# mhamilton723/STEGO

Hardware: AMD Instinct MI355X
Metric: image-pairs/sec through correspondence loss, B=32 224^2, ViT-S/8 (higher is better)
Workload: dtype f16x3 (f32 inputs / outputs / accumulation; products of the feature and code correlations and of the backward's code GEMMs as fp16 hi+lo splits, 22-bit, on the matrix cores - error vs fp64 in the fp32 class, bounded by tests on adversarial inputs); 1 GPU; vits8_224: B=32/GPU, C=384, 28x28 map, K=70, S=11, 5 negatives, self+KNN+random correlation loss, forward+backward; global_batch=32, parallelism=dp1, launch=eager, input_sets_rotated=4, layout=channels-last strided views (as DinoFeaturizer)

## Files before the change

stego_amd/csrc/corr_bwd.hip:

```cpp
#include "corr_common.h"
#include "host_util.h"

namespace stego {

constexpr int LDG = 130;
constexpr int SMB_NRM = 0;
constexpr int SMB_AN = SMB_NRM + 2 * TP * 4;

template <int NT>
__device__ __forceinline__ void normalize_bwd_store(f32x4 (&d)[2][NT], const float* __restrict__ Cn, int ldk,
                                                    const float* __restrict__ nrm, float* __restrict__ dt_out,
                                                    int K, int KQ, int lane, int wave)
{
    const int cl = lane & 15, rg = lane >> 4;
#pragma unroll
    for (int mt = 0; mt < 2; ++mt) {
#pragma unroll
        for (int reg = 0; reg < 4; ++reg) {
            const int pt = 32 * wave + 16 * mt + 4 * rg + reg;
            float cn[NT];
            float dot = 0.f;
#pragma unroll
            for (int nt = 0; nt < NT; ++nt) {
                const int ch = 16 * nt + cl;
// ... 150 lines not shown
    if (!sameAB) normalize_bwd_store<NT>(dA, An, ldk, nrm, dtA, K, prm.KQ, lane, wave);
    for (int kk = 0; kk < kend; kk += 4) {
        const int k = kk + kq;
        float gt[2], an[NT];
        gt[0] = G[k * LDG + row0];
        gt[1] = G[k * LDG + row0 + 16];
#pragma unroll
        for (int nt = 0; nt < NT; ++nt) an[nt] = An[k * ldk + 16 * nt + cl];
#pragma unroll
        for (int nt = 0; nt < NT; ++nt) {
            dB[0][nt] = __builtin_amdgcn_mfma_f32_16x16x4f32(gt[0], an[nt], dB[0][nt], 0, 0, 0);
            dB[1][nt] = __builtin_amdgcn_mfma_f32_16x16x4f32(gt[1], an[nt], dB[1][nt], 0, 0, 0);
        }
    }
    if (stamp_on) ts[2] = __builtin_amdgcn_s_memrealtime();
    if (sameAB) {
#pragma unroll
        for (int mt = 0; mt < 2; ++mt)
#pragma unroll
            for (int nt = 0; nt < NT; ++nt) dA[mt][nt] += dB[mt][nt];
        normalize_bwd_store<NT>(dA, An, ldk, nrm, dtA, K, prm.KQ, lane, wave);
    } else {
        normalize_bwd_store<NT>(dB, Bn, ldk, nrm + TP, dtA + (size_t)TP * ldk, K, prm.KQ, lane, wave);
    }
    if (stamp_on) ts[3] = __builtin_amdgcn_s_memrealtime();
}

template <int NT>
__global__ void __launch_bounds__(NTHREADS) corr_bwd_tile_kernel(const BwdParams prm)
{
    extern __shared__ __attribute__((aligned(16))) unsigned char smem[];
    bwd_tile_body<NT>(prm, (int)blockIdx.x, smem);
}

constexpr int HB_LDR = 136;
constexpr int SMH_NRM = 0;
constexpr int SMH_CT = 1280;

typedef _Float16 f16x4 __attribute__((ext_vector_type(4)));

constexpr int HW_WAVES = 8;
constexpr int HW_THREADS = 64 * HW_WAVES;
constexpr int HW_NP = TP / (16 * HW_WAVES);
template <int NT>
__device__ __forceinline__ void normalize_bwd_store_t(f32x4 (&d)[NT][HW_NP], const float* __restrict__ Cn, int ldk,
                                                      const float* __restrict__ nrm, float* __restrict__ dt_out,
                                                      int K, int KQ, int lane, int wave, bool wt = false)
{
    const int cl = lane & 15, kq = lane >> 4;
#pragma unroll
    for (int np = 0; np < HW_NP; ++np) {
        const int pt = 16 * (HW_NP * wave + np) + cl;
        f32x4 cn[NT];
        float dot = 0.f;
#pragma unroll
        for (int mc = 0; mc < NT; ++mc) {
            const int ch0 = 16 * mc + 4 * kq;
            cn[mc] = *reinterpret_cast<const f32x4*>(Cn + (size_t)pt * ldk + ch0);
#pragma unroll
            for (int reg = 0; reg < 4; ++reg) {
                if (ch0 + reg >= K) cn[mc][reg] = 0.f;
                dot += cn[mc][reg] * (ch0 + reg < K ? d[mc][np][reg] : 0.f);
            }
        }
        dot += __shfl_xor(dot, 16, 64);
        dot += __shfl_xor(dot, 32, 64);
        const float nr = nrm[pt];
        const bool big = nr > 1e-10f;
        const float inv = 1.f / fmaxf(nr, 1e-10f);
#pragma unroll
        for (int mc = 0; mc < NT; ++mc) {
            const int ch0 = 16 * mc + 4 * kq;
            if (ch0 < KQ) {
                f32x4 v;
#pragma unroll
                for (int reg = 0; reg < 4; ++reg) {
                    const float dn = d[mc][np][reg];
                    v[reg] = big ? (dn - cn[mc][reg] * dot) * inv : dn * inv;
                    if (ch0 + reg >= K) v[reg] = 0.f;
                }
                float* dst = dt_out + (size_t)pt * ldk + ch0;
                if (wt) asm volatile("global_store_dwordx4 %0, %1, off sc1" :: "v"(dst), "v"(v) : "memory");
                else *reinterpret_cast<f32x4*>(dst) = v;
            }
        }
    }
}

template <int NT, bool DENSE>
__device__ __forceinline__ void bwd_tile_h_body(const BwdParams& prm, const int tile, unsigned char* smem)
{
    constexpr int NTG = NT <= 5 ? NT : (NT + 1) / 2;
    constexpr int NG = (NT + NTG - 1) / NTG;
    constexpr int CTR = 16 * NTG;
    float* nrm = reinterpret_cast<float*>(smem + SMH_NRM);
    float* red = nrm + 2 * TP;
    half_t* CT = reinterpret_cast<half_t*>(smem + SMH_CT);
    half_t* Gh = CT + 4 * CTR * HB_LDR;
    half_t* Gl = Gh + TP * HB_LDR;

    const int tid = threadIdx.x, lane = tid & 63;
    const int wave = __builtin_amdgcn_readfirstlane(tid >> 6);
    const int B = prm.B, P = prm.P, K = prm.K, ldk = prm.LDK;
    const int b = tile % B, p = tile / B;
    const bool sameAB = p == 0;
    const int sA = b;
    const int sB = p == 0 ? b : p * B + b;
    const float* csA = prm.cs + (size_t)sA * TP * ldk;
    const float* csB = prm.cs + (size_t)sB * TP * ldk;

    unsigned long long* ts = reinterpret_cast<unsigned long long*>(prm.dt + (size_t)prm.n_sets * B * 2 * TP * ldk) + 4096 + (size_t)tile * 4;
    const bool stamp_on = (prm.debug & 8) && tid == 0 && tile < 1024;
    if (stamp_on) ts[0] = __builtin_amdgcn_s_memrealtime();

    const int P2 = P * P;
    const size_t t0 = p < 2 ? (size_t)b * P2 : ((size_t)(p - 2) * B + b) * P2;
    const float* wp = prm.saved_w + ((size_t)p * B + b) * P2;
    const float* glp = wp;
    bool has_gl = false;
    float gl_b = 0.f;
    if (p >= 2) {
        if (prm.g_neg_loss) {
            if (DENSE && prm.g_neg_loss_stride > 0) { glp = prm.g_neg_loss + t0; has_gl = true; }
            else if (prm.g_neg_loss_stride < 0) gl_b = prm.g_neg_loss[0] * (1.f / ((float)B * (float)P2 * (float)prm.n_neg));
            else gl_b = prm.g_neg_loss[0];
        }
    } else {
        const float* gs = p == 0 ? prm.g_intra : prm.g_inter;
        if (gs) gl_b = gs[0] * (1.f / ((float)B * (float)P2));
    }
    const float* gcd = !DENSE ? nullptr : (p == 0 ? prm.g_intra_cd : (p == 1 ? prm.g_inter_cd : prm.g_neg_cd));
    const bool has_gc = gcd != nullptr;
    const float* gcp = has_gc ? gcd + t0 : wp;
    const float om = prm.saved_mean[p];

    constexpr int RB = TP / HW_WAVES;
    constexpr int c4n = CTR / 4;
    constexpr int NIT = ((TP / 2) * c4n + HW_THREADS - 1) / HW_THREADS;
    float wv[RB][2], glv[RB][2], gcv[RB][2];
    f32x4 r0[2][NIT], r1[2][NIT];
    auto load_codes = [&](int grp) {
#pragma unroll
        for (int side = 0; side < 2; ++side) {
            const float* src = ((side == 0 || sameAB) ? csA : csB) + grp * CTR;
#pragma unroll
            for (int it = 0; it < NIT; ++it) {
                const int i = (prm.debug & 16) ? 0 : min(tid + it * HW_THREADS, (TP / 2) * c4n - 1);
                const int pp = i / c4n, c4 = i - pp * c4n;
                r0[side][it] = *reinterpret_cast<const f32x4*>(src + (size_t)(2 * pp) * ldk + 4 * c4);
                r1[side][it] = *reinterpret_cast<const f32x4*>(src + (size_t)(2 * pp + 1) * ldk + 4 * c4);
            }
        }
    };
    auto convert_codes = [&](int grp) {
#pragma unroll
        for (int side = 0; side < 2; ++side) {
            if (side == 1 && sameAB) break;
            half_t* dh = CT + (size_t)(2 * side) * CTR * HB_LDR;
            half_t* dl = dh + CTR * HB_LDR;
#pragma unroll
            for (int it = 0; it < NIT; ++it) {
                const int i = tid + it * HW_THREADS;
                if (i < (TP / 2) * c4n) {
                    const int pp = i / c4n, c4 = i - pp * c4n;
#pragma unroll
                    for (int e = 0; e < 4; ++e) {
                        const int ch = 4 * c4 + e;
                        const bool in = grp * CTR + ch < K;
                        unsigned h, l;
                        split_f16_pair(in ? r0[side][it][e] : 0.f, in ? r1[side][it][e] : 0.f, h, l);
                        const int col = (((pp >> 1) ^ (ch >> 4)) << 2) + 2 * (pp & 1);
                        *reinterpret_cast<unsigned*>(dh + ch * HB_LDR + col) = h;
                        *reinterpret_cast<unsigned*>(dl + ch * HB_LDR + col) = l;
                    }
                }
            }
        }
    };
    {
        const int c0 = min(2 * lane, P - 1), c1 = min(2 * lane + 1, P - 1);
#pragma unroll
        for (int j = 0; j < RB; ++j) {
            const int r = (prm.debug & 4) ? 0 : min(wave + HW_WAVES * j, P - 1);
            wv[j][0] = wp[r * P + c0];
            wv[j][1] = wp[r * P + c1];
        }
        if (has_gl) {
#pragma unroll
            for (int j = 0; j < RB; ++j) {
                const int r = min(wave + HW_WAVES * j, P - 1);
                glv[j][0] = glp[r * P + c0];
                glv[j][1] = glp[r * P + c1];
            }
        }
        if (has_gc) {
#pragma unroll
            for (int j = 0; j < RB; ++j) {
                const int r = min(wave + HW_WAVES * j, P - 1);
                gcv[j][0] = gcp[r * P + c0];
                gcv[j][1] = gcp[r * P + c1];
            }
        }
        load_codes(0);
    }
    if (tid < 2 * TP) nrm[tid] = prm.nrm[(size_t)(tid < TP ? sA : sB) * TP + (tid & (TP - 1))];
    float gmax = 0.f;
#pragma unroll
    for (int j = 0; j < RB; ++j) {
        const int r = wave + HW_WAVES * j;
#pragma unroll
        for (int h = 0; h < 2; ++h) {
            const unsigned wb = __builtin_bit_cast(unsigned, wv[j][h]);
            const float w = __builtin_bit_cast(float, wb & ~1u);
            float g = (wb & 1u) ? -(w + om) * (has_gl ? glv[j][h] : gl_b) : 0.f;
            if (has_gc) g += gcv[j][h];
            g = (r < P && 2 * lane + h < P) ? g : 0.f;
            wv[j][h] = g;
            gmax = fmaxf(gmax, fabsf(g));
        }
    }
    float tmax;
    if constexpr (DENSE) {
#pragma unroll
        for (int m = 32; m >= 1; m >>= 1) gmax = fmaxf(gmax, __shfl_xor(gmax, m, 64));
        if (lane == 0) red[wave] = gmax;
        __syncthreads();
        tmax = 0.f;
#pragma unroll
        for (int w2 = 0; w2 < HW_WAVES; ++w2) tmax = fmaxf(tmax, red[w2]);
    } else {
        tmax = 4.f * fabsf(gl_b);
    }
    float sc_tile = 1.f, inv_tile = 1.f;
    if (tmax > 0.f && tmax < 3.0e38f) {
        const int e = __builtin_amdgcn_frexp_expf(tmax);
        sc_tile = __builtin_ldexpf(1.f, -e);
        inv_tile = __builtin_ldexpf(1.f, e);
    }
#pragma unroll
    for (int j = 0; j < RB; ++j) {
        const int r = wave + HW_WAVES * j;
        unsigned hi, lo;
        split_f16_pair(wv[j][0] * sc_tile, wv[j][1] * sc_tile, hi, lo);
        *reinterpret_cast<unsigned*>(Gh + r * HB_LDR + 2 * lane) = hi;
        *reinterpret_cast<unsigned*>(Gl + r * HB_LDR + 2 * lane) = lo;
    }

    const int cl = lane & 15, kq = lane >> 4;
    half_t* ATh = CT;
    half_t* ATl = CT + CTR * HB_LDR;
    half_t* BTh = sameAB ? ATh : CT + 2 * CTR * HB_LDR;
    half_t* BTl = sameAB ? ATl : CT + 3 * CTR * HB_LDR;
    float* dtA = prm.dt + ((size_t)tile * 2 + 0) * TP * ldk;
    const bool skip = (prm.debug & 1) || tmax == 0.f;

    const bool early_dB = NG == 1 && !sameAB && !skip && !(prm.debug & 2048);
    f32x4 dAt[NT][HW_NP], dBt[NT][HW_NP];
#pragma unroll
    for (int mc = 0; mc < NT; ++mc)
#pragma unroll
        for (int np = 0; np < HW_NP; ++np) { dAt[mc][np] = f32x4{0.f, 0.f, 0.f, 0.f}; dBt[mc][np] = f32x4{0.f, 0.f, 0.f, 0.f}; }

#pragma unroll
    for (int grp = 0; grp < NG; ++grp) {
        if (grp > 0) {
            __syncthreads();
            load_codes(grp);
        }
        convert_codes(grp);
        __syncthreads();
        if (stamp_on && grp == 0) ts[1] = __builtin_amdgcn_s_memrealtime();
        if (skip) continue;
        auto gemm_dA = [&]() {
            {
                const int ra = cl * HB_LDR + 4 * kq;
                const int rg = (16 * HW_NP * wave + cl) * HB_LDR + 4 * kq;
#pragma unroll 2
                for (int kk = 0; kk < TP; kk += 16) {
                    f16x4 ah[NTG], al[NTG], bh[HW_NP], bl[HW_NP];
#pragma unroll
                    for (int mc = 0; mc < NTG; ++mc) {
                        const int ks = ((((kk >> 2) + kq) ^ mc) << 2) - 4 * kq;
                        ah[mc] = *reinterpret_cast<const f16x4*>(BTh + ra + 16 * mc * HB_LDR + ks);
                        al[mc] = *reinterpret_cast<const f16x4*>(BTl + ra + 16 * mc * HB_LDR + ks);
                    }
#pragma unroll
                    for (int np = 0; np < HW_NP; ++np) {
                        bh[np] = *reinterpret_cast<const f16x4*>(Gh + rg + 16 * np * HB_LDR + kk);
                        bl[np] = *reinterpret_cast<const f16x4*>(Gl + rg + 16 * np * HB_LDR + kk);
                    }
#pragma unroll
                    for (int term = 0; term < 3; ++term)
#pragma unroll
                        for (int mc = 0; mc < NTG; ++mc)
#pragma unroll
                            for (int np = 0; np < HW_NP; ++np)
                                if (grp * NTG + mc < NT)
                                    dAt[grp * NTG + mc][np] = __builtin_amdgcn_mfma_f32_16x16x16f16(
                                        term == 2 ? al[mc] : ah[mc], term == 1 ? bl[np] : bh[np], dAt[grp * NTG + mc][np], 0, 0, 0);
                }
            }
        };
        auto gemm_dB = [&]() {
            {
                const int ra = cl * HB_LDR + 4 * kq;
                const int gt = (4 * kq + (cl >> 2)) * HB_LDR + 16 * HW_NP * wave + 4 * (cl & 3);
                typedef __fp16 fp16x4v __attribute__((__vector_size__(4 * sizeof(__fp16))));
                typedef __attribute__((address_space(3))) fp16x4v* lds_tr_ptr;
#pragma unroll 2
                for (int kk = 0; kk < TP; kk += 16) {
                    f16x4 ah[NTG], al[NTG], bh[HW_NP], bl[HW_NP];
#pragma unroll
                    for (int mc = 0; mc < NTG; ++mc) {
                        const int ks = ((((kk >> 2) + kq) ^ mc) << 2) - 4 * kq;
                        ah[mc] = *reinterpret_cast<const f16x4*>(ATh + ra + 16 * mc * HB_LDR + ks);
                        al[mc] = *reinterpret_cast<const f16x4*>(ATl + ra + 16 * mc * HB_LDR + ks);
                    }
#pragma unroll
                    for (int np = 0; np < HW_NP; ++np) {
                        const fp16x4v th = __builtin_amdgcn_ds_read_tr16_b64_v4f16((lds_tr_ptr)(Gh + gt + kk * HB_LDR + 16 * np));
                        const fp16x4v tl = __builtin_amdgcn_ds_read_tr16_b64_v4f16((lds_tr_ptr)(Gl + gt + kk * HB_LDR + 16 * np));
                        __builtin_memcpy(&bh[np], &th, 8);
                        __builtin_memcpy(&bl[np], &tl, 8);
                    }
#pragma unroll
                    for (int term = 0; term < 3; ++term)
#pragma unroll
                        for (int mc = 0; mc < NTG; ++mc)
#pragma unroll
                            for (int np = 0; np < HW_NP; ++np)
                                if (grp * NTG + mc < NT)
                                    dBt[grp * NTG + mc][np] = __builtin_amdgcn_mfma_f32_16x16x16f16(
                                        term == 2 ? al[mc] : ah[mc], term == 1 ? bl[np] : bh[np], dBt[grp * NTG + mc][np], 0, 0, 0);
                }
            }
        };
        if (early_dB) {
            gemm_dB();
#pragma unroll
            for (int mc = 0; mc < NT; ++mc)
#pragma unroll
                for (int np = 0; np < HW_NP; ++np) dBt[mc][np] *= inv_tile;
            normalize_bwd_store_t<NT>(dBt, csB, ldk, nrm + TP, dtA + (size_t)TP * ldk, K, prm.KQ, lane, wave, true);
            gemm_dA();
        } else {
            gemm_dA();
            gemm_dB();
        }
    }
    if (stamp_on) ts[2] = __builtin_amdgcn_s_memrealtime();
#pragma unroll
    for (int mc = 0; mc < NT; ++mc)
#pragma unroll
        for (int np = 0; np < HW_NP; ++np) { dAt[mc][np] *= inv_tile; if (!early_dB) dBt[mc][np] *= inv_tile; }
    if (sameAB) {
#pragma unroll
        for (int mc = 0; mc < NT; ++mc)
#pragma unroll
            for (int np = 0; np < HW_NP; ++np) dAt[mc][np] += dBt[mc][np];
        normalize_bwd_store_t<NT>(dAt, csA, ldk, nrm, dtA, K, prm.KQ, lane, wave);
    } else {
        normalize_bwd_store_t<NT>(dAt, csA, ldk, nrm, dtA, K, prm.KQ, lane, wave);
        if (!early_dB) normalize_bwd_store_t<NT>(dBt, csB, ldk, nrm + TP, dtA + (size_t)TP * ldk, K, prm.KQ, lane, wave);
    }
    if (stamp_on) ts[3] = __builtin_amdgcn_s_memrealtime();
}

template <int NT, bool DENSE>
__global__ void __launch_bounds__(HW_THREADS) corr_bwd_tile_h_kernel(const BwdParams prm)
{
    extern __shared__ __attribute__((aligned(16))) unsigned char smem[];
    bwd_tile_h_body<NT, DENSE>(prm, (int)blockIdx.x, smem);
}

constexpr int UNS_THREADS = 512;
constexpr int UNS_SETS_PER_ROUND = UNS_THREADS / TP;
constexpr int UNS_MAX_RT = 8;
constexpr int UNS_ROW_CAP = 192;
constexpr int UNS_MAX_CONTRIB = 1024;

struct UnsRowEntry {
    int dtoff;
    int x01;
    float wa, wb;
};

__global__ void __launch_bounds__(UNS_THREADS) corr_unsample_kernel(const BwdParams prm, const int RT, const int n_bands,
                                                                   const int acc_bytes)
{
    extern __shared__ __attribute__((aligned(16))) unsigned char smem[];
    float* acc = reinterpret_cast<float*>(smem);
    int* ctab = reinterpret_cast<int*>(smem + acc_bytes);
    UnsRowEntry* wl = reinterpret_cast<UnsRowEntry*>(smem + acc_bytes + UNS_MAX_CONTRIB * 4);
    int* cnt = reinterpret_cast<int*>(smem + acc_bytes + UNS_MAX_CONTRIB * 4 + UNS_MAX_RT * UNS_ROW_CAP * (int)sizeof(UnsRowEntry));
    int& s_nc = cnt[UNS_MAX_RT];
    const int tid = threadIdx.x, lane = tid & 63;
    const int wave = __builtin_amdgcn_readfirstlane(tid >> 6);
    const int B = prm.B, P = prm.P, K = prm.K, W = prm.W, H = prm.H, ldk = prm.LDK;
    const bool direct = prm.mode == 1;
    int bid = blockIdx.x;
    const int band = bid % n_bands; bid /= n_bands;
    const int j = bid % B;
    const int dest = bid / B;
    const int r0 = band * RT, r1 = min(H, r0 + RT);
    const int band_elems = (r1 - r0) * W * K;
    const int side_elems = TP * ldk;
    for (int e = tid; e < band_elems; e += UNS_THREADS) acc[e] = 0.f;

    const int n_own = (!direct && dest == 0) ? prm.n_sets : 1;
    if (wave == 0) {
        int nc = n_own;
        if (!direct && dest == 0) {
            for (int i = 0; i < prm.n_neg; ++i)
                for (int b0 = 0; b0 < B; b0 += 64) {
                    const int bb = b0 + lane;
                    const bool m = bb < B && (int)prm.perms[(size_t)i * B + bb] == j;
                    const unsigned long long mask = __ballot(m);
                    const int pre = __builtin_popcountll(mask & ((1ull << lane) - 1ull));
                    if (m && nc + pre < UNS_MAX_CONTRIB) ctab[nc + pre] = (2 + i) * B + bb;
                    nc += __builtin_popcountll(mask);
                }
            if (nc > UNS_MAX_CONTRIB) nc = UNS_MAX_CONTRIB;
        }
        if (lane == 0) s_nc = nc;
    }
    __syncthreads();
    const int NC = s_nc;
    

    for (int c0 = 0; c0 < NC; c0 += UNS_SETS_PER_ROUND) {
        if (tid < UNS_MAX_RT) cnt[tid] = 0;
        __syncthreads();
        {
            const int c = c0 + (tid >> 7), q = tid & (TP - 1);
            if (c < NC && q < P && !(prm.debug & 2)) {
                int s, tile0, side;
                if (c < n_own) {
                    if (direct) { s = dest * B + j; tile0 = j; side = dest; }
                    else if (dest == 1) { s = B + j; tile0 = B + j; side = 1; }
                    else { s = j; tile0 = c * B + j; side = 0; }
                } else { s = ctab[c]; tile0 = s; side = 1; }
                const int4 yx = prm.tapyx[(size_t)s * TP + q];
                const float4 w = prm.tapw[(size_t)s * TP + q];
                const int dtoff = (tile0 * 2 + side) * side_elems + q * ldk;
#pragma unroll
                for (int hrow = 0; hrow < 2; ++hrow) {
                    const int y = (hrow ? yx.z : yx.x) >> 16;
                    const float wa = hrow ? w.z : w.x, wb = hrow ? w.w : w.y;
                    if (y < r0 || y >= r1 || (wa == 0.f && wb == 0.f)) continue;
                    if (hrow == 1 && y == (yx.x >> 16)) continue;
                    const int xa = (hrow ? yx.z : yx.x) & 0xffff, xb = (hrow ? yx.w : yx.y) & 0xffff;
                    const int row = y - r0;
                    const int slot = atomicAdd(&cnt[row], 1);
                    if (slot < UNS_ROW_CAP) {
                        UnsRowEntry e;
                        e.dtoff = dtoff; e.x01 = xa | (xb << 16); e.wa = wa; e.wb = wb;
                        wl[row * UNS_ROW_CAP + slot] = e;
                    } else {
                        for (int ch = 0; ch < K; ++ch) {
                            const float v = prm.dt[dtoff + ch];
                            if (wa != 0.f) atomicAdd(&acc[(row * W + xa) * K + ch], wa * v);
                            if (wb != 0.f) atomicAdd(&acc[(row * W + xb) * K + ch], wb * v);
                        }
                    }
                }
            }
        }
        __syncthreads();
        if (wave < r1 - r0) {
            const int count = min(cnt[wave], UNS_ROW_CAP);
            const UnsRowEntry* list = wl + wave * UNS_ROW_CAP;
            float* arow = acc + wave * W * K;
            constexpr int UB = 16;
            const int cA = min(lane, K - 1), cB = min(64 + lane, K - 1);
            const bool hasA = lane < K, hasB = 64 + lane < K;
            float* dummy = acc + (acc_bytes >> 2) - 4 * 64 + lane;
            for (int e0 = 0; e0 < count; e0 += UB) {
                float v0[UB], v1[UB], wa[UB], wb[UB];
                int x01[UB];
#pragma unroll
                for (int u = 0; u < UB; ++u) {
                    const UnsRowEntry en = list[min(e0 + u, count - 1)];
                    const bool on = e0 + u < count;
                    x01[u] = en.x01; wa[u] = on ? en.wa : 0.f; wb[u] = on ? en.wb : 0.f;
                    v0[u] = prm.dt[en.dtoff + cA];
                    v1[u] = prm.dt[en.dtoff + cB];
                }
                if (!(prm.debug & 16)) {
#pragma unroll
                    for (int u = 0; u < UB; ++u) {
                        const int xa = x01[u] & 0xffff, xb = x01[u] >> 16;
                        const bool two = xb != xa;
                        float* pa0 = hasA ? arow + xa * K + lane : dummy;
                        float* pb0 = (hasA && two) ? arow + xb * K + lane : dummy + 64;
                        float* pa1 = hasB ? arow + xa * K + 64 + lane : dummy + 128;
                        float* pb1 = (hasB && two) ? arow + xb * K + 64 + lane : dummy + 192;
                        const float a0 = *pa0, b0 = *pb0, a1 = *pa1, b1 = *pb1;
                        *pa0 = a0 + wa[u] * v0[u];
                        *pb0 = b0 + wb[u] * v0[u];
                        *pa1 = a1 + wa[u] * v1[u];
                        *pb1 = b1 + wb[u] * v1[u];
                    }
                }
            }
        }
        __syncthreads();
    }
    float* out = (dest == 0 ? prm.d_code : prm.d_code_pos) + ((size_t)j * H + r0) * W * K;
    for (int e = tid; e < band_elems; e += UNS_THREADS) out[e] = acc[e];
}


constexpr int UR_WAVES = 3;
constexpr int UR_GROUP = 6;
constexpr int UR_CAP = UR_GROUP * TP;
// ... 90 lines not shown
                int yx0[UR_GROUP][2];
#pragma unroll
                for (int g = 0; g < UR_GROUP; ++g) {
                    const int2 it = items[min(it_pos + g, n_items - 1)];
#pragma unroll
                    for (int h = 0; h < 2; ++h)
                        yx0[g][h] = reinterpret_cast<const int*>(prm.tapyx + (size_t)it.x * TP + h * 64 + lane)[0];
                }
#pragma unroll
                for (int g = 0; g < UR_GROUP; ++g) {
#pragma unroll
                    for (int h = 0; h < 2; ++h) {
                        const int q = h * 64 + lane;
                        const int y0 = yx0[g][h] >> 16, x0 = yx0[g][h] & 0xffff;
                        const bool hit = it_pos + g < n_items && q < P && (y0 == r || y0 + 1 == r);
#pragma unroll
                        for (int m = 0; m < MT; ++m) {
                            const bool mine = hit && ((x0 >> 4) == m || x0 == 16 * m - 1);
                            const unsigned long long mask = __ballot(mine);
                            if (mine) wl[m * UR_CAP + cnt[m] + lane_prefix(mask)] = (it_pos + g) << 7 | q;
                            cnt[m] += __builtin_popcountll(mask);
                        }
                    }
                }
            }
            __builtin_amdgcn_wave_barrier();
            int off[MT + 1];
            off[0] = 0;
#pragma unroll
            for (int m = 0; m < MT; ++m) off[m + 1] = off[m] + ((cnt[m] + 3) & ~3);
            int count = off[MT];

            if (prm.debug & 128) count = 0;
            for (int e0 = 0; e0 < count; e0 += 4 * UR_EG) {
                float bv[UR_EG][UR_NT];
                int meta[UR_EG];
#pragma unroll
                for (int g = 0; g < UR_EG; ++g) {
                    const int eg = min(e0 + 4 * g, count - 4);
                    int m = 0;
#pragma unroll
                    for (int mm = 1; mm < MT; ++mm) m += eg >= off[mm] ? 1 : 0;
                    int base = 0, n = cnt[0], o = 0;
#pragma unroll
                    for (int mm = 1; mm < MT; ++mm) if (m == mm) { base = mm * UR_CAP; n = cnt[mm]; o = off[mm]; }
                    const int pk = wl[base + min(eg - o + k4, n - 1)];
                    const int2 it = items[pk >> 7];
                    const int q = pk & (TP - 1);
                    const unsigned rowoff = (unsigned)(it.y + q * ldk);
#pragma unroll
                    for (int nt = 0; nt < UR_NT; ++nt) bv[g][nt] = prm.dt[rowoff + (unsigned)cch[nt]];
                    meta[g] = tap_words[(unsigned)(it.x * TP + q) * 4u + meta_off];
                }
                __builtin_amdgcn_sched_barrier(0);
                if (prm.debug & 64) {
                    float sum = 0.f;
#pragma unroll
                    for (int g = 0; g < UR_EG; ++g) {
                        sum += __builtin_bit_cast(float, meta[g]);
#pragma unroll
                        for (int nt = 0; nt < UR_NT; ++nt) sum += bv[g][nt];
                    }
                    acc[0][0][0] += sum;
                    continue;
                }
#pragma unroll
                for (int g = 0; g < UR_EG; ++g) {
                    const int eg = e0 + 4 * g;
                    if (eg < count) {
                        int m = 0;
#pragma unroll
                        for (int mm = 1; mm < MT; ++mm) m += eg >= off[mm] ? 1 : 0;
                        int n = cnt[0], o = 0;
#pragma unroll
                        for (int mm = 1; mm < MT; ++mm) if (m == mm) { n = cnt[mm]; o = off[mm]; }
                        const int yx = __shfl(meta[g], grp_lane0, 64);
                        const int x0 = yx & 0xffff;
                        const int low = (yx >> 16) != r ? 2 : 0;
                        float wa = __builtin_bit_cast(float, __shfl(meta[g], grp_lane0 + 4 + low, 64));
                        float wb = __builtin_bit_cast(float, __shfl(meta[g], grp_lane0 + 5 + low, 64));
                        if (eg - o + k4 >= n) { wa = 0.f; wb = 0.f; }
#pragma unroll
                        for (int mt = 0; mt < MT; ++mt) {
                            if (m == mt) {
                                const int dx = 16 * mt + l16 - x0;
                                const float a = dx == 0 ? wa : (dx == 1 ? wb : 0.f);
#pragma unroll
                                for (int nt = 0; nt < UR_NT; ++nt)
                                    acc[mt][nt] = __builtin_amdgcn_mfma_f32_16x16x4f32(a, bv[g][nt], acc[mt][nt], 0, 0, 0);
                            }
                        }
                    }
                }
            }
            __builtin_amdgcn_wave_barrier();
        }
    }

    float* out = (dest == 0 ? prm.d_code : prm.d_code_pos) + ((size_t)j * H + r) * W * K;
    if (!heavy) {
#pragma unroll
        for (int mt = 0; mt < MT; ++mt)
#pragma unroll
            for (int reg = 0; reg < 4; ++reg) {
                const int x = 16 * mt + 4 * k4 + reg;
#pragma unroll
                for (int nt = 0; nt < UR_NT; ++nt) {
                    const int ch = 16 * nt + l16;
                    if (x < W && ch < K) __builtin_nontemporal_store(acc[mt][nt][reg], out + (size_t)x * K + ch);
                }
            }
        return;
    }
    f32x4* red = reinterpret_cast<f32x4*>(wl_raw);
#pragma unroll
    for (int mt = 0; mt < MT; ++mt) {
        __syncthreads();
#pragma unroll
        for (int nt = 0; nt < UR_NT; ++nt) red[(wave * UR_NT + nt) * 64 + lane] = acc[mt][nt];
        __syncthreads();
#pragma unroll
        for (int t = 0; t < (UR_NT + UR_WAVES - 1) / UR_WAVES; ++t) {
            const int nt = wave + UR_WAVES * t;
            if (nt < UR_NT) {
                f32x4 v = red[nt * 64 + lane];
#pragma unroll
                for (int w2 = 1; w2 < UR_WAVES; ++w2) v += red[(w2 * UR_NT + nt) * 64 + lane];
                const int ch = 16 * nt + l16;
#pragma unroll
                for (int reg = 0; reg < 4; ++reg) {
                    const int x = 16 * mt + 4 * k4 + reg;
                    if (x < W && ch < K) __builtin_nontemporal_store(v[reg], out + (size_t)x * K + ch);
                }
            }
        }
    }
    if (stamp_on) ts[2 * blockIdx.x + 1] = __builtin_amdgcn_s_memrealtime();
}

constexpr int BF_ITEM_CAP = 1032;
constexpr int BF_MAXH = 64, BF_MAXMT = 4;
constexpr int BF_NKEY = 2 * BF_MAXH * BF_MAXMT;
constexpr int UL_CAP0 = 63, UL_CAP1 = 15;
constexpr int UL_SLOT0 = 16 * (UL_CAP0 + 1), UL_SLOT1 = 16 * (UL_CAP1 + 1);
constexpr int BFS_ITEMS = 0;
constexpr int BFS_HIST = BFS_ITEMS + BF_ITEM_CAP * 8;
constexpr int BFS_OVF = BFS_HIST + HW_WAVES * BF_NKEY * 4;
constexpr int BFS_SCAN = BFS_OVF + BF_NKEY * 4;
constexpr int BFS_MISC = BFS_SCAN + 64;
constexpr int BF_LDS_BYTES = BFS_MISC + 64;
static_assert(BF_NKEY % HW_THREADS == 0 && BF_NKEY % NTHREADS == 0, "whole keys per thread in the prefix");

typedef unsigned int bu32x4 __attribute__((ext_vector_type(4)));

__device__ __forceinline__ __amdgpu_buffer_rsrc_t bf_rsrc(const void* p, unsigned bytes)
{
    return __builtin_amdgcn_make_buffer_rsrc(const_cast<void*>(p), 0, bytes, 0x00020000);
}

template <int NW>
__device__ __forceinline__ void bwd_builder_role(const BwdParams& prm, const int bi, unsigned char* smem)
{
    int2* items = reinterpret_cast<int2*>(smem + BFS_ITEMS);
    unsigned* hist = reinterpret_cast<unsigned*>(smem + BFS_HIST);
    unsigned* ovf = reinterpret_cast<unsigned*>(smem + BFS_OVF);
    unsigned* scan = reinterpret_cast<unsigned*>(smem + BFS_SCAN);
    int* misc = reinterpret_cast<int*>(smem + BFS_MISC);
    const int tid = threadIdx.x, lane = tid & 63;
    const int wave = __builtin_amdgcn_readfirstlane(tid >> 6);
    const int B = prm.B, P = prm.P, H = prm.H, W = prm.W, ldk = prm.LDK;
    const int MT = (W + 15) >> 4;
    const int side_elems = TP * ldk;
    const unsigned EPI = 4u * (unsigned)P;
    const unsigned light0 = (unsigned)(B * H * MT) * UL_SLOT0;
    const __amdgpu_buffer_rsrc_t pool = bf_rsrc(prm.upool, prm.upool_bytes);
    const __amdgpu_buffer_rsrc_t slots = bf_rsrc(prm.uslots, prm.uslots_bytes);
    unsigned long long* ts = reinterpret_cast<unsigned long long*>(prm.dt + (size_t)prm.n_sets * B * 2 * side_elems) + 2048 + 2 * bi;
    const bool stamp_on = (prm.debug & 8) && tid == 0 && bi < 512;
    if (stamp_on) ts[0] = __builtin_amdgcn_s_memrealtime();
    unsigned* myhist = hist + wave * BF_NKEY;

    for (int j = bi; j < B; j += prm.n_build) {
        __syncthreads();
        if (wave == 0) {
            const int n_own = prm.n_sets;
            for (int u = lane; u < n_own; u += 64) items[u] = make_int2(j, ((u * B + j) * 2 + 0) * side_elems);
            int n_seen = 0, below = 0;
            const int n_negc = prm.n_neg * B;
            for (int t0 = 0; t0 < n_negc; t0 += 64) {
                const int t = t0 + lane;
                const long long pv = t < n_negc ? prm.perms[t] : -1;
                const bool m = (int)pv == j && t < n_negc;
                const unsigned long long mask = __ballot(m);
                const int s = 2 * B + t;
                if (m) items[n_own + n_seen + lane_prefix(mask)] = make_int2(s, (s * 2 + 1) * side_elems);
                n_seen += __builtin_popcountll(mask);
                below += __builtin_popcountll(__ballot(t < n_negc && (int)pv < j));
            }
            const int n0 = n_own + n_seen;
            if (lane == 0) {
                items[n0] = make_int2(B + j, ((B + j) * 2 + 1) * side_elems);
                misc[0] = n0;
                misc[1] = (int)(EPI * (unsigned)(prm.n_sets * j + below));
                misc[2] = (int)(EPI * (unsigned)(prm.n_sets * B + n_negc + j));
            }
        }
        for (int i = tid; i < NW * BF_NKEY; i += (64 * NW)) hist[i] = 0u;
        __syncthreads();
        const int n0 = misc[0], n_ih = 2 * (n0 + 1);
        const unsigned slab0 = (unsigned)misc[1], slab1 = (unsigned)misc[2];
        auto point_keys = [&](int dest, int q, int wd, int (&key)[4]) {
            const int y0 = wd >> 16, x0 = wd & 0xffff;
            const int b0 = x0 >> 4, b1 = (x0 & 15) == 15 && b0 + 1 < MT ? b0 + 1 : -1;
            const bool v = q < P;
            const int r0 = (dest * H + y0) * BF_MAXMT, r1 = r0 + BF_MAXMT;
            key[0] = v ? r0 + b0 : -1;
            key[1] = v && b1 >= 0 ? r0 + b1 : -1;
            key[2] = v && y0 + 1 < H ? r1 + b0 : -1;
            key[3] = v && y0 + 1 < H && b1 >= 0 ? r1 + b1 : -1;
        };
        for (int ih0 = wave; ih0 < n_ih; ih0 += 4 * NW) {
            int wd[4];
#pragma unroll
            for (int u = 0; u < 4; ++u) {
                const int ih = min(ih0 + u * NW, n_ih - 1), it = ih >> 1, q = (ih & 1) * 64 + lane;
                wd[u] = reinterpret_cast<const int*>(prm.tapyx + (size_t)items[it].x * TP + q)[0];
            }
#pragma unroll
            for (int u = 0; u < 4; ++u) {
                const int ih = ih0 + u * NW;
                if (ih < n_ih) {
                    int key[4];
                    point_keys((ih >> 1) >= n0, (ih & 1) * 64 + lane, wd[u], key);
#pragma unroll
                    for (int c = 0; c < 4; ++c)
                        if (key[c] >= 0) __hip_atomic_fetch_add(myhist + key[c], 1u, __ATOMIC_RELAXED, __HIP_MEMORY_SCOPE_WORKGROUP);
                }
            }
        }
        __syncthreads();
        {
            constexpr int KPT = BF_NKEY / (64 * NW);
            const int kd1 = H * BF_MAXMT;
            unsigned c[KPT][NW], tot[KPT], over[KPT], osum = 0u;
#pragma unroll
            for (int i = 0; i < KPT; ++i) {
                const int key = tid * KPT + i;
                tot[i] = 0u;
#pragma unroll
                for (int w = 0; w < NW; ++w) { c[i][w] = hist[w * BF_NKEY + key]; tot[i] += c[i][w]; }
                const unsigned cap = key >= kd1 ? UL_CAP1 : UL_CAP0;
                over[i] = tot[i] > cap ? tot[i] - cap : 0u;
                osum += over[i];
            }
            unsigned inc = osum;
#pragma unroll
            for (int d = 1; d < 64; d <<= 1) {
                const unsigned o = (unsigned)__shfl_up((int)inc, d, 64);
                if (lane >= d) inc += o;
            }
            if (lane == 63) scan[wave] = inc;
            __syncthreads();
            unsigned base = inc - osum;
#pragma unroll
            for (int w = 0; w < NW; ++w) base += w < wave ? scan[w] : 0u;
            unsigned kb[KPT];
#pragma unroll
            for (int i = 0; i < KPT; ++i) { kb[i] = base; base += over[i]; }
#pragma unroll
            for (int i = 0; i < KPT; ++i)
                if (tid * KPT + i == kd1) scan[NW] = kb[i];
            __syncthreads();
#pragma unroll
            for (int i = 0; i < KPT; ++i) {
                const int key = tid * KPT + i;
                const bool d1 = key >= kd1;
                const unsigned ostart = d1 ? slab1 + (kb[i] - scan[NW]) : slab0 + kb[i];
                ovf[key] = ostart;
                const int rm = key - (d1 ? kd1 : 0), m = rm & (BF_MAXMT - 1);
                if (key < 2 * kd1 && m < MT) {
                    const unsigned ui = (unsigned)((j * H + (rm >> 2)) * MT + m);
                    __builtin_amdgcn_raw_buffer_store_b128(bu32x4{tot[i], ostart, 0u, 0u}, slots, d1 ? light0 + ui * UL_SLOT1 : ui * UL_SLOT0, 0, 0);
                }
                unsigned run = 0u;
#pragma unroll
                for (int w = 0; w < NW; ++w) { hist[w * BF_NKEY + key] = run; run += c[i][w]; }
            }
        }
        __syncthreads();
        const int kd1 = H * BF_MAXMT;
        for (int ih0 = wave; ih0 < n_ih; ih0 += 4 * NW) {
            int wd[4];
            float4 w4[4];
#pragma unroll
            for (int u = 0; u < 4; ++u) {
                const int ih = min(ih0 + u * NW, n_ih - 1), it = ih >> 1, q = (ih & 1) * 64 + lane;
                const size_t e = (size_t)items[it].x * TP + q;
                wd[u] = reinterpret_cast<const int*>(prm.tapyx + e)[0];
                w4[u] = prm.tapw[e];
            }
#pragma unroll
            for (int u = 0; u < 4; ++u) {
                const int ih = ih0 + u * NW;
                if (ih < n_ih) {
                    const int it = ih >> 1, q = (ih & 1) * 64 + lane;
                    const bool d1 = it >= n0;
                    int key[4];
                    point_keys(d1, q, wd[u], key);
                    bu32x4 ent;
                    ent[0] = (unsigned)(items[it].y + q * ldk);
                    ent[1] = (unsigned)(wd[u] & 0xffff);
#pragma unroll
                    for (int c = 0; c < 4; ++c)
                        if (key[c] >= 0) {
                            const unsigned pos = __hip_atomic_fetch_add(myhist + key[c], 1u, __ATOMIC_RELAXED, __HIP_MEMORY_SCOPE_WORKGROUP);
                            ent[2] = __builtin_bit_cast(unsigned, c >= 2 ? w4[u].z : w4[u].x);
                            ent[3] = __builtin_bit_cast(unsigned, c >= 2 ? w4[u].w : w4[u].y);
                            const int rm = key[c] - (d1 ? kd1 : 0);
                            const unsigned ui = (unsigned)((j * H + (rm >> 2)) * MT + (rm & (BF_MAXMT - 1)));
                            const unsigned cap = d1 ? UL_CAP1 : UL_CAP0;
                            if (pos < cap) __builtin_amdgcn_raw_buffer_store_b128(ent, slots, (d1 ? light0 + ui * UL_SLOT1 : ui * UL_SLOT0) + 16u * (1u + pos), 0, 0);
                            else __builtin_amdgcn_raw_buffer_store_b128(ent, pool, (ovf[key[c]] + (pos - cap)) * 16u, 0, 0);
                        }
                }
            }
        }
    }
    if (stamp_on) ts[1] = __builtin_amdgcn_s_memrealtime();
}

template <int NT>
__global__ void __launch_bounds__(HW_THREADS) corr_bwd_tile_build_kernel(const BwdParams prm)
{
    extern __shared__ __attribute__((aligned(16))) unsigned char smem[];
    const int w = blockIdx.x;
    if (w < prm.n_build) bwd_builder_role<HW_WAVES>(prm, w, smem);
    else bwd_tile_h_body<NT, false>(prm, w - prm.n_build, smem);
}

template <int NT>
__global__ void __launch_bounds__(NTHREADS) corr_bwd_tile32_build_kernel(const BwdParams prm)
{
    extern __shared__ __attribute__((aligned(16))) unsigned char smem[];
    const int w = blockIdx.x;
    if (w < prm.n_build) bwd_builder_role<NTHREADS / 64>(prm, w, smem);
    else bwd_tile_body<NT>(prm, w - prm.n_build, smem);
}

constexpr int UL_WAVES = 4;
template <int NQ, int TAIL>
__global__ void __launch_bounds__(64 * UL_WAVES) corr_unsample_list_kernel(const BwdParams prm)
{
    constexpr int NA = 4 * NQ + TAIL;
    constexpr int EG0 = (UL_CAP0 + 1) / 4, EG1 = (UL_CAP1 + 1) / 4;
    const int lane = threadIdx.x & 63;
    const int wave = __builtin_amdgcn_readfirstlane(threadIdx.x >> 6);
    const int B = prm.B, H = prm.H, W = prm.W, K = prm.K, ldk = prm.LDK;
    const int MT = (W + 15) >> 4;
    const int n_pairs = B * H * MT;
    int k;
    {
        const int upi = H * MT, wpi = (upi + UL_WAVES - 1) / UL_WAVES;
        const int x = blockIdx.x & 7, sl = blockIdx.x >> 3;
        const int j = (sl / wpi) * 8 + x, u = (sl % wpi) * UL_WAVES + wave;
        if (j >= B || u >= upi) return;
        k = j * upi + u;
    }
    if (k >= n_pairs) return;
    const int l16 = lane & 15, k4 = lane >> 4;
    const __amdgpu_buffer_rsrc_t pool = bf_rsrc(prm.upool, prm.upool_bytes);
    const __amdgpu_buffer_rsrc_t slots = bf_rsrc(prm.uslots, prm.uslots_bytes);
    const __amdgpu_buffer_rsrc_t dtr = bf_rsrc(prm.dt, prm.dt_bytes);
    const unsigned light0 = (unsigned)n_pairs * UL_SLOT0;
    unsigned long long* ts = reinterpret_cast<unsigned long long*>(prm.dt + (size_t)prm.n_sets * B * 2 * TP * ldk) + 2 * blockIdx.x;
    const bool stamp_on = (prm.debug & 8) && threadIdx.x == 0 && blockIdx.x < 1024;
    if (stamp_on) ts[0] = __builtin_amdgcn_s_memrealtime();
    const int m = k % MT, jr = k / MT;

    bu32x4 s0 = __builtin_amdgcn_raw_buffer_load_b128(slots, (unsigned)k * UL_SLOT0 + 16u * lane, 0, 0);
    bu32x4 s1 = __builtin_amdgcn_raw_buffer_load_b128(slots, light0 + (unsigned)k * UL_SLOT1 + 16u * (lane & 15), 0, 0);
    const unsigned n0 = __builtin_amdgcn_readfirstlane(s0[0]), o0 = __builtin_amdgcn_readfirstlane(s0[1]);
    const unsigned n1 = __builtin_amdgcn_readfirstlane(s1[0]), o1 = __builtin_amdgcn_readfirstlane(s1[1]);

    f32x4 acc[2][NA];
#pragma unroll
    for (int u = 0; u < 2; ++u)
#pragma unroll
        for (int a = 0; a < NA; ++a) acc[u][a] = f32x4{0.f, 0.f, 0.f, 0.f};

    struct Rows { f32x4 q[NQ]; float t[TAIL > 0 ? TAIL : 1]; };
    auto issue = [&](const bu32x4& ent, int first, int n, auto& rows, auto ng_tag) {
        constexpr int NG = decltype(ng_tag)::value;
#pragma unroll
        for (int g = 0; g < NG; ++g) {
            if (4 * g < n) {
                const int e = min(4 * g + k4, n - 1);
                const unsigned row = (unsigned)__shfl((int)ent[0], first + e, 64);
#pragma unroll
                for (int qd = 0; qd < NQ; ++qd)
                    rows[g].q[qd] = __builtin_bit_cast(f32x4, __builtin_amdgcn_raw_buffer_load_b128(dtr, (row + 64u * qd + 4u * l16) * 4u, 0, 0));
#pragma unroll
                for (int t = 0; t < TAIL; ++t)
                    rows[g].t[t] = __builtin_bit_cast(float, __builtin_amdgcn_raw_buffer_load_b32(dtr, (row + (unsigned)min(64 * NQ + 16 * t + l16, ldk - 1)) * 4u, 0, 0));
            }
        }
    };
    auto consume = [&](const bu32x4& ent, int first, int n, auto& rows, f32x4 (&ac)[NA], auto ng_tag) {
        constexpr int NG = decltype(ng_tag)::value;
#pragma unroll
        for (int g = 0; g < NG; ++g) {
            if (4 * g < n) {
                const int e = min(4 * g + k4, n - 1);
                const int x0 = __shfl((int)ent[1], first + e, 64);
                float wa = __builtin_bit_cast(float, __shfl((int)ent[2], first + e, 64));
                float wb = __builtin_bit_cast(float, __shfl((int)ent[3], first + e, 64));
                if (4 * g + k4 >= n) { wa = 0.f; wb = 0.f; }
                const int dx = 16 * m + l16 - x0;
                const float a = dx == 0 ? wa : (dx == 1 ? wb : 0.f);
#pragma unroll
                for (int qd = 0; qd < NQ; ++qd)
#pragma unroll
                    for (int c = 0; c < 4; ++c)
                        ac[4 * qd + c] = __builtin_amdgcn_mfma_f32_16x16x4f32(a, rows[g].q[qd][c], ac[4 * qd + c], 0, 0, 0);
#pragma unroll
                for (int t = 0; t < TAIL; ++t)
                    ac[4 * NQ + t] = __builtin_amdgcn_mfma_f32_16x16x4f32(a, rows[g].t[t], ac[4 * NQ + t], 0, 0, 0);
            }
        }
    };
    {
        Rows r0[EG0], r1[EG1];
        const int c0 = (int)min(n0, (unsigned)UL_CAP0), c1 = (int)min(n1, (unsigned)UL_CAP1);
        issue(s0, 1, c0, r0, std::integral_constant<int, EG0>());
        issue(s1, 1, c1, r1, std::integral_constant<int, EG1>());
        __builtin_amdgcn_sched_barrier(0);
        consume(s0, 1, c0, r0, acc[0], std::integral_constant<int, EG0>());
        consume(s1, 1, c1, r1, acc[1], std::integral_constant<int, EG1>());
    }
#pragma unroll
    for (int u = 0; u < 2; ++u) {
        const int rest = u ? (int)n1 - UL_CAP1 : (int)n0 - UL_CAP0;
        const unsigned ob = u ? o1 : o0;
        for (int e0 = 0; e0 < rest; e0 += 64) {
            const int n = min(64, rest - e0);
            const bu32x4 ent = __builtin_amdgcn_raw_buffer_load_b128(pool, (ob + (unsigned)(e0 + min(lane, n - 1))) * 16u, 0, 0);
            Rows r[16];
            issue(ent, 0, n, r, std::integral_constant<int, 16>());
            __builtin_amdgcn_sched_barrier(0);
            consume(ent, 0, n, r, acc[u], std::integral_constant<int, 16>());
        }
    }
#pragma unroll
    for (int u = 0; u < 2; ++u) {
        float* out = (u == 0 ? prm.d_code : prm.d_code_pos) + (size_t)jr * W * K;
#pragma unroll
        for (int reg = 0; reg < 4; ++reg) {
            const int x = 16 * m + 4 * k4 + reg;
            if (x < W) {
                float* px = out + (size_t)x * K;
#pragma unroll
                for (int qd = 0; qd < NQ; ++qd) {
                    const int ch = 64 * qd + 4 * l16;
                    const f32x4 v = f32x4{acc[u][4 * qd][reg], acc[u][4 * qd + 1][reg], acc[u][4 * qd + 2][reg], acc[u][4 * qd + 3][reg]};
                    if (ch + 3 < K) {
                        typedef f32x4 f32x4_a4 __attribute__((aligned(4)));
                        __builtin_nontemporal_store(v, reinterpret_cast<f32x4_a4*>(px + ch));
                    } else {
#pragma unroll
                        for (int c = 0; c < 4; ++c)
                            if (ch + c < K) __builtin_nontemporal_store(v[c], px + ch + c);
                    }
                }
#pragma unroll
                for (int t = 0; t < TAIL; ++t) {
                    const int ch = 64 * NQ + 16 * t + l16;
                    if (ch < K) __builtin_nontemporal_store(acc[u][4 * NQ + t][reg], px + ch);
                }
            }
        }
    }
    if (stamp_on) ts[1] = __builtin_amdgcn_s_memrealtime();
}

bool bwd_lists_supported(const BwdParams& prm)
{
    const int nt = (prm.KQ + 15) / 16;
    const bool dense = prm.g_intra_cd || prm.g_inter_cd || prm.g_neg_cd || (prm.g_neg_loss && prm.g_neg_loss_stride > 0);
    if ((prm.debug & 512) && nt > 5) return false;
    return prm.uslots && prm.upool && prm.mode == 0 && !dense && prm.H <= BF_MAXH && prm.W <= 16 * BF_MAXMT &&
           !(prm.debug & (32 | 1024)) && (size_t)prm.n_sets * prm.B * 2 * TP * prm.LDK < ((size_t)1 << 30);
}

hipError_t launch_corr_bwd_lists(const BwdParams& prm_in, hipStream_t stream)
{
    BwdParams prm = prm_in;
    const int nt = (prm.KQ + 15) / 16;
    const int ntg = nt <= 5 ? nt : (nt + 1) / 2;
    const bool split = !(prm.debug & 512) && (prm.precision == PREC_F16X3 || nt > 5);
    int lds = split ? SMH_CT + (4 * 16 * ntg + 2 * TP) * HB_LDR * 2 : SMB_AN + 2 * TP * prm.LDK * 4 + TP * LDG * 4;
    if (lds < BF_LDS_BYTES) lds = BF_LDS_BYTES;
    const int n_tiles = prm.n_sets * prm.B;
    prm.n_build = prm.B < 32 ? prm.B : 32;
    {
        const dim3 grid(prm.n_build + n_tiles);
#define STEGO_BWDL_CASE(N)                                                                                        \
    case N: {                                                                                                     \
        hipError_t ea = ensure_dynamic_lds(reinterpret_cast<const void*>(&corr_bwd_tile_build_kernel<N>), lds);   \
        if (ea != hipSuccess) return ea;                                                                          \
        hipLaunchKernelGGL((corr_bwd_tile_build_kernel<N>), grid, dim3(HW_THREADS), lds, stream, prm);            \
        break;                                                                                                    \
    }
#define STEGO_BWDL32_CASE(N)                                                                                      \
    case N: {                                                                                                     \
        hipError_t ea = ensure_dynamic_lds(reinterpret_cast<const void*>(&corr_bwd_tile32_build_kernel<N>), lds); \
        if (ea != hipSuccess) return ea;                                                                          \
        hipLaunchKernelGGL((corr_bwd_tile32_build_kernel<N>), grid, dim3(NTHREADS), lds, stream, prm);            \
        break;                                                                                                    \
    }
        if (split) {
            switch (nt) {
                STEGO_BWDL_CASE(1)
                STEGO_BWDL_CASE(2)
                STEGO_BWDL_CASE(3)
                STEGO_BWDL_CASE(4)
                STEGO_BWDL_CASE(5)
                STEGO_BWDL_CASE(6)
                STEGO_BWDL_CASE(7)
                default:
                STEGO_BWDL_CASE(8)
            }
        } else {
            switch (nt) {
                STEGO_BWDL32_CASE(1)
                STEGO_BWDL32_CASE(2)
                STEGO_BWDL32_CASE(3)
                STEGO_BWDL32_CASE(4)
                default:
                STEGO_BWDL32_CASE(5)
            }
        }
#undef STEGO_BWDL_CASE
#undef STEGO_BWDL32_CASE
        hipError_t e = hipGetLastError();
        if (e != hipSuccess) return e;
    }
    const int upi = prm.H * ((prm.W + 15) >> 4), wpi = (upi + UL_WAVES - 1) / UL_WAVES;
    const dim3 grid(((prm.B + 7) / 8) * 8 * wpi), block(64 * UL_WAVES);
    if (prm.K <= 64) hipLaunchKernelGGL((corr_unsample_list_kernel<1, 0>), grid, block, 0, stream, prm);
    else if (prm.K <= 80) hipLaunchKernelGGL((corr_unsample_list_kernel<1, 1>), grid, block, 0, stream, prm);
    else hipLaunchKernelGGL((corr_unsample_list_kernel<2, 0>), grid, block, 0, stream, prm);
    return hipGetLastError();
}

hipError_t launch_corr_bwd(const BwdParams& prm, hipStream_t stream)
{
    if (bwd_lists_supported(prm)) return launch_corr_bwd_lists(prm, stream);
    {
        const int cside = TP * prm.LDK * 4;
        const int nt = (prm.KQ + 15) / 16;
        const bool split = prm.mode == 0 && !(prm.debug & 512) && (prm.precision == PREC_F16X3 || nt > 5);
        const int ntg = nt <= 5 ? nt : (nt + 1) / 2;
        const bool dense = prm.g_intra_cd || prm.g_inter_cd || prm.g_neg_cd || (prm.g_neg_loss && prm.g_neg_loss_stride > 0);
        const int lds = split ? SMH_CT + (4 * 16 * ntg + 2 * TP) * HB_LDR * 2 : SMB_AN + 2 * cside + TP * LDG * 4;
        const dim3 grid(prm.n_sets * prm.B), block(NTHREADS);
#define STEGO_BWD_CASE(N)                                                                                         \
    case N: {                                                                                                     \
        if (split && dense) {                                                                                     \
            hipError_t ea = ensure_dynamic_lds(reinterpret_cast<const void*>(&corr_bwd_tile_h_kernel<N, true>), lds);   \
            if (ea != hipSuccess) return ea;                                                                      \
            hipLaunchKernelGGL((corr_bwd_tile_h_kernel<N, true>), grid, dim3(HW_THREADS), lds, stream, prm);      \
        } else if (split) {                                                                                       \
            hipError_t ea = ensure_dynamic_lds(reinterpret_cast<const void*>(&corr_bwd_tile_h_kernel<N, false>), lds);  \
            if (ea != hipSuccess) return ea;                                                                      \
            hipLaunchKernelGGL((corr_bwd_tile_h_kernel<N, false>), grid, dim3(HW_THREADS), lds, stream, prm);     \
        } else {                                                                                                  \
            hipError_t ea = ensure_dynamic_lds(reinterpret_cast<const void*>(&corr_bwd_tile_kernel<N>), lds);    \
            if (ea != hipSuccess) return ea;                                                                      \
            hipLaunchKernelGGL((corr_bwd_tile_kernel<N>), grid, block, lds, stream, prm);                         \
        }                                                                                                         \
        break;                                                                                                    \
    }
        if (nt > 5 && !split) return hipErrorInvalidValue;
        if (nt > 5) {
#define STEGO_BWD_WIDE(N)                                                                                         \
    case N: {                                                                                                     \
        if (dense) {                                                                                              \
            hipError_t ea = ensure_dynamic_lds(reinterpret_cast<const void*>(&corr_bwd_tile_h_kernel<N, true>), lds);   \
            if (ea != hipSuccess) return ea;                                                                      \
            hipLaunchKernelGGL((corr_bwd_tile_h_kernel<N, true>), grid, dim3(HW_THREADS), lds, stream, prm);      \
        } else {                                                                                                  \
            hipError_t ea = ensure_dynamic_lds(reinterpret_cast<const void*>(&corr_bwd_tile_h_kernel<N, false>), lds);  \
            if (ea != hipSuccess) return ea;                                                                      \
            hipLaunchKernelGGL((corr_bwd_tile_h_kernel<N, false>), grid, dim3(HW_THREADS), lds, stream, prm);     \
        }                                                                                                         \
        break;                                                                                                    \
    }
// ... 53 lines not shown
```

Measured before the change: 404,200 image-pairs/s.

## Defer B-side code conversion behind early dB GEMM and prefetch overflow entries

In the backward tile kernel, when the dB GEMM runs early, only the A-side codes are converted to fp16 hi/lo before the first barrier. The B-side conversion now happens after the dB store, which shortens the path to the first GEMM. The norm load is hoisted above the weight loads. In the scatter consumer, when NQ==1 the first batch of overflow pool entries is loaded and issued together with the in-slot rows, hiding pool-load latency. A debug-gated write-through store option and extra timestamp probes are also added. The cost is higher register pressure from holding B codes and the extra prefetched rows.

```diff
diff --git a/stego_amd/csrc/corr_bwd.hip b/stego_amd/csrc/corr_bwd.hip
--- a/stego_amd/csrc/corr_bwd.hip
+++ b/stego_amd/csrc/corr_bwd.hip
@@ -326,10 +326,9 @@
             }
         }
     };
-    auto convert_codes = [&](int grp) {
-#pragma unroll
-        for (int side = 0; side < 2; ++side) {
-            if (side == 1 && sameAB) break;
+    auto convert_side = [&](int grp, auto side_tag) {
+        {
+            constexpr int side = decltype(side_tag)::value;
             half_t* dh = CT + (size_t)(2 * side) * CTR * HB_LDR;
             half_t* dl = dh + CTR * HB_LDR;
 #pragma unroll
@@ -351,6 +350,12 @@
             }
         }
     };
+    auto convert_codes = [&](int grp) {
+        convert_side(grp, std::integral_constant<int, 0>());
+        if (!sameAB) convert_side(grp, std::integral_constant<int, 1>());
+    };
+    float nrm_v = 0.f;
+    if (tid < 2 * TP) nrm_v = prm.nrm[(size_t)(tid < TP ? sA : sB) * TP + (tid & (TP - 1))];
     {
         const int c0 = min(2 * lane, P - 1), c1 = min(2 * lane + 1, P - 1);
 #pragma unroll
@@ -377,7 +382,7 @@
         }
         load_codes(0);
     }
-    if (tid < 2 * TP) nrm[tid] = prm.nrm[(size_t)(tid < TP ? sA : sB) * TP + (tid & (TP - 1))];
+    if (tid < 2 * TP) nrm[tid] = nrm_v;
     float gmax = 0.f;
 #pragma unroll
     for (int j = 0; j < RB; ++j) {
@@ -429,6 +434,8 @@
     const bool skip = (prm.debug & 1) || tmax == 0.f;
 
     const bool early_dB = NG == 1 && !sameAB && !skip && !(prm.debug & 2048);
+    const bool late_B = early_dB && !(prm.debug & 4096);
+    unsigned long long* tsb = ts - (4096 + (size_t)tile * 4) + 3072 + tile;
     f32x4 dAt[NT][HW_NP], dBt[NT][HW_NP];
 #pragma unroll
     for (int mc = 0; mc < NT; ++mc)
@@ -441,9 +448,11 @@
             __syncthreads();
             load_codes(grp);
         }
-        convert_codes(grp);
+        if (late_B) convert_side(grp, std::integral_constant<int, 0>());
+        else convert_codes(grp);
         __syncthreads();
         if (stamp_on && grp == 0) ts[1] = __builtin_amdgcn_s_memrealtime();
+        if (stamp_on && grp == 0 && !late_B) tsb[0] = ts[1];
         if (skip) continue;
         auto gemm_dA = [&]() {
             {
@@ -516,6 +525,13 @@
 #pragma unroll
                 for (int np = 0; np < HW_NP; ++np) dBt[mc][np] *= inv_tile;
             normalize_bwd_store_t<NT>(dBt, csB, ldk, nrm + TP, dtA + (size_t)TP * ldk, K, prm.KQ, lane, wave, true);
+            if (late_B) {
+#pragma unroll
+                for (int it = 0; it < NIT; ++it) asm volatile("" : "+v"(r0[1][it]), "+v"(r1[1][it]));
+                convert_side(grp, std::integral_constant<int, 1>());
+                __syncthreads();
+                if (stamp_on) tsb[0] = __builtin_amdgcn_s_memrealtime();
+            }
             gemm_dA();
         } else {
             gemm_dA();
@@ -534,7 +550,7 @@
             for (int np = 0; np < HW_NP; ++np) dAt[mc][np] += dBt[mc][np];
         normalize_bwd_store_t<NT>(dAt, csA, ldk, nrm, dtA, K, prm.KQ, lane, wave);
     } else {
-        normalize_bwd_store_t<NT>(dAt, csA, ldk, nrm, dtA, K, prm.KQ, lane, wave);
+        normalize_bwd_store_t<NT>(dAt, csA, ldk, nrm, dtA, K, prm.KQ, lane, wave, (prm.debug & 16384) != 0);
         if (!early_dB) normalize_bwd_store_t<NT>(dBt, csB, ldk, nrm + TP, dtA + (size_t)TP * ldk, K, prm.KQ, lane, wave);
     }
     if (stamp_on) ts[3] = __builtin_amdgcn_s_memrealtime();
@@ -931,6 +947,7 @@
 static_assert(BF_NKEY % HW_THREADS == 0 && BF_NKEY % NTHREADS == 0, "whole keys per thread in the prefix");
 
 typedef unsigned int bu32x4 __attribute__((ext_vector_type(4)));
+constexpr int BF_AUX_SC1 = 16;
 
 __device__ __forceinline__ __amdgpu_buffer_rsrc_t bf_rsrc(const void* p, unsigned bytes)
 {
@@ -958,6 +975,7 @@
     const bool stamp_on = (prm.debug & 8) && tid == 0 && bi < 512;
     if (stamp_on) ts[0] = __builtin_amdgcn_s_memrealtime();
     unsigned* myhist = hist + wave * BF_NKEY;
+    const bool wthru = (prm.debug & 8192) != 0;
 
     for (int j = bi; j < B; j += prm.n_build) {
         __syncthreads();
@@ -1059,7 +1077,9 @@
                 const int rm = key - (d1 ? kd1 : 0), m = rm & (BF_MAXMT - 1);
                 if (key < 2 * kd1 && m < MT) {
                     const unsigned ui = (unsigned)((j * H + (rm >> 2)) * MT + m);
-                    __builtin_amdgcn_raw_buffer_store_b128(bu32x4{tot[i], ostart, 0u, 0u}, slots, d1 ? light0 + ui * UL_SLOT1 : ui * UL_SLOT0, 0, 0);
+                    const unsigned so = d1 ? light0 + ui * UL_SLOT1 : ui * UL_SLOT0;
+                    if (wthru) __builtin_amdgcn_raw_buffer_store_b128(bu32x4{tot[i], ostart, 0u, 0u}, slots, so, 0, BF_AUX_SC1);
+                    else __builtin_amdgcn_raw_buffer_store_b128(bu32x4{tot[i], ostart, 0u, 0u}, slots, so, 0, 0);
                 }
                 unsigned run = 0u;
 #pragma unroll
@@ -1098,8 +1118,14 @@
                             const int rm = key[c] - (d1 ? kd1 : 0);
                             const unsigned ui = (unsigned)((j * H + (rm >> 2)) * MT + (rm & (BF_MAXMT - 1)));
                             const unsigned cap = d1 ? UL_CAP1 : UL_CAP0;
-                            if (pos < cap) __builtin_amdgcn_raw_buffer_store_b128(ent, slots, (d1 ? light0 + ui * UL_SLOT1 : ui * UL_SLOT0) + 16u * (1u + pos), 0, 0);
-                            else __builtin_amdgcn_raw_buffer_store_b128(ent, pool, (ovf[key[c]] + (pos - cap)) * 16u, 0, 0);
+                            const unsigned so = (d1 ? light0 + ui * UL_SLOT1 : ui * UL_SLOT0) + 16u * (1u + pos), po = (ovf[key[c]] + (pos - cap)) * 16u;
+                            if (wthru) {
+                                if (pos < cap) __builtin_amdgcn_raw_buffer_store_b128(ent, slots, so, 0, BF_AUX_SC1);
+                                else __builtin_amdgcn_raw_buffer_store_b128(ent, pool, po, 0, BF_AUX_SC1);
+                            } else {
+                                if (pos < cap) __builtin_amdgcn_raw_buffer_store_b128(ent, slots, so, 0, 0);
+                                else __builtin_amdgcn_raw_buffer_store_b128(ent, pool, po, 0, 0);
+                            }
                         }
                 }
             }
@@ -1207,20 +1233,38 @@
             }
         }
     };
+    constexpr bool AHEAD = NQ == 1;
+    constexpr int AHG = TAIL ? 14 : 16;
+    const bool ahead = AHEAD && !(prm.debug & 256);
     {
         Rows r0[EG0], r1[EG1];
         const int c0 = (int)min(n0, (unsigned)UL_CAP0), c1 = (int)min(n1, (unsigned)UL_CAP1);
+        const int pa = ahead ? min(max((int)n0 - UL_CAP0, 0), 4 * AHG) : 0;
+        bu32x4 pent = bu32x4{0u, 0u, 0u, 0u};
+        if (AHEAD && pa > 0) {
+            pent = __builtin_amdgcn_raw_buffer_load_b128(pool, (o0 + (unsigned)min(lane, pa - 1)) * 16u, 0, 0);
+            asm volatile("" : "+v"(pent[0]), "+v"(pent[1]), "+v"(pent[2]), "+v"(pent[3]));
+        }
         issue(s0, 1, c0, r0, std::integral_constant<int, EG0>());
         issue(s1, 1, c1, r1, std::integral_constant<int, EG1>());
-        __builtin_amdgcn_sched_barrier(0);
-        consume(s0, 1, c0, r0, acc[0], std::integral_constant<int, EG0>());
-        consume(s1, 1, c1, r1, acc[1], std::integral_constant<int, EG1>());
+        if constexpr (AHEAD) {
+            Rows rp[AHG];
+            issue(pent, 0, pa, rp, std::integral_constant<int, AHG>());
+            __builtin_amdgcn_sched_barrier(0);
+            consume(s0, 1, c0, r0, acc[0], std::integral_constant<int, EG0>());
+            consume(s1, 1, c1, r1, acc[1], std::integral_constant<int, EG1>());
+            consume(pent, 0, pa, rp, acc[0], std::integral_constant<int, AHG>());
+        } else {
+            __builtin_amdgcn_sched_barrier(0);
+            consume(s0, 1, c0, r0, acc[0], std::integral_constant<int, EG0>());
+            consume(s1, 1, c1, r1, acc[1], std::integral_constant<int, EG1>());
+        }
     }
 #pragma unroll
     for (int u = 0; u < 2; ++u) {
         const int rest = u ? (int)n1 - UL_CAP1 : (int)n0 - UL_CAP0;
         const unsigned ob = u ? o1 : o0;
-        for (int e0 = 0; e0 < rest; e0 += 64) {
+        for (int e0 = (u == 0 && ahead) ? 4 * AHG : 0; e0 < rest; e0 += 64) {
             const int n = min(64, rest - e0);
             const bu32x4 ent = __builtin_amdgcn_raw_buffer_load_b128(pool, (ob + (unsigned)(e0 + min(lane, n - 1))) * 16u, 0, 0);
             Rows r[16];
```

New measurement: 393,400 image-pairs/s. 0.973x the previous value.
